# apple/ml-neuman

Hardware: AMD Instinct MI355X
Metric: rays_per_sec (800x800 frame, 128 samples/ray coarse + 128 importance, NeuMan background NeRF) (higher is better)
Workload: dtype coarse (sampling) pass: split-fp16 hi+lo MFMA x3, f32 accumulate; fine (shading) pass: per-row-scaled int16 as two int8 limbs on the i8 MFMA x3, exact int32 accumulate, encodings on split bf16

## Files before the change

include/neuman_hip.h:

```cpp
#ifndef NEUMAN_HIP_H
#define NEUMAN_HIP_H

#include <stdint.h>

#ifdef __cplusplus
extern "C" {
#endif

#define NM_OK 0
#define NM_ERR_ARG (-1)
#define NM_ERR_HIP (-2)
#define NM_ERR_UNSUPPORTED (-3)

#define NM_ABI_VERSION 1

typedef void* nm_stream_t;

#define NM_PREC_FP32 0
#define NM_PREC_BF16X3 1
#define NM_PREC_BF16 2
#define NM_PREC_I8X3 3
#define NM_PREC_FP16X3 4

#define NM_PE_POSENC 0
// ... 50 lines not shown
int nm_mlp_create(const nm_mlp_desc* desc, const float* const* host_params, const float* host_pos_tab,
                  const float* host_dir_tab, nm_mlp_t* out);
int nm_mlp_destroy(nm_mlp_t mlp);

int nm_mlp_forward(nm_mlp_t mlp, const float* pts, const float* dirs, int64_t n, int precision,
                   float sigma_scale, float* out, nm_stream_t stream);
int nm_mlp_refresh_f16(nm_mlp_t mlp, const float* const* dev_params, nm_stream_t stream);
int nm_mlp_forward_save(nm_mlp_t mlp, const float* pts, const float* dirs, int64_t n, float* save_h, float* save_hv,
                        float* out, nm_stream_t stream);
int nm_mlp_forward_save_bits(nm_mlp_t mlp, const float* pts, const float* dirs, int64_t n, float* save_h, float* save_hv,
                             uint32_t* save_bits, float* out, nm_stream_t stream);
int64_t nm_mlp_backward_chain_workspace_floats(int64_t n);
int nm_mlp_backward_chain(nm_mlp_t mlp, const float* const* dev_params, const float* dz_top, const float* d_feat, const float* d_raw,
                          const float* acts, const uint32_t* relu_bits, int64_t n, float* dz_out, float* bias_grads, float* workspace,
                          int64_t workspace_floats, nm_stream_t stream);
int nm_mlp_forward_save16(nm_mlp_t mlp, const float* pts, const float* dirs, int64_t n, uint16_t* save_h16, float* save_feat, uint16_t* save_feat16,
                          float* save_hv, uint32_t* save_bits, uint32_t* save_hvbits, uint16_t* save_x0h, uint16_t* save_d0h, float* out,
                          nm_stream_t stream);
int nm_mlp_backward_chain16(nm_mlp_t mlp, const float* const* dev_params, const float* d_feat, const float* d_raw, const uint32_t* relu_bits,
                            int64_t n, const float* amax, uint16_t* dz16, uint16_t* dfeat16, float* dz32_layer5, float* dz32_layer0,
                            float* bias_grads, float* workspace, int64_t workspace_floats, nm_stream_t stream);
int nm_mlp_backward_plain16(nm_mlp_t mlp, const float* const* dev_params, const float* d_out, const uint32_t* relu_bits, int64_t n, const float* amax,
                            uint16_t* dz16, float* dz32_layer5, float* dz32_layer0, float* bias_grads, float* workspace, int64_t workspace_floats,
                            nm_stream_t stream);
int nm_mlp_backward_net16(nm_mlp_t mlp, const float* const* dev_params, const float* d_raw, const float* d_feat_add, const uint32_t* relu_bits,
                          const uint32_t* hv_bits, int64_t n, const float* amax, uint16_t* dz16, uint16_t* dfeat16, uint16_t* dhv16, float* dz32_layer5, float* dz32_layer0,
                          float* dhv32, float* bias_grads, float* workspace, int64_t workspace_floats, nm_stream_t stream);
int nm_mlp_forward_rays(nm_mlp_t mlp, const float* origin, const float* direction, const float* z_vals,
                        int64_t R, int S, int precision, float sigma_scale, float* out, nm_stream_t stream);
#define NM_LIVE_CHUNK_SAMPLES (1 << 21)
int64_t nm_mlp_forward_rays_live_workspace_bytes(int64_t R, int S, int64_t chunk_samples);
int nm_mlp_forward_rays_live(nm_mlp_t mlp, const float* origin, const float* direction, const float* z_vals, int64_t R, int S, int precision,
                             float sigma_scale, float* out, void* workspace, int64_t workspace_bytes, int64_t chunk_samples, nm_stream_t stream);
int nm_mlp_sigma_rays(nm_mlp_t mlp, const float* origin, const float* direction, const float* z_vals,
                      int64_t R, int S, int precision, float sigma_scale, float* out, nm_stream_t stream);
int nm_mlp_forward_ray_chunk(nm_mlp_t mlp, const float* origin, const float* direction, const float* z_vals, int S_total,
                             const int32_t* ray_idx, const int32_t* n_rays_dev, int64_t n_rays, int s0, int S, int precision,
                             float sigma_scale, float* out, nm_stream_t stream);
int nm_mlp_sigma_ray_chunk(nm_mlp_t mlp, const float* origin, const float* direction, const float* z_vals, int S_total,
                           const int32_t* ray_idx, const int32_t* n_rays_dev, int64_t n_rays, int s0, int S, int precision,
                           float sigma_scale, float* out, nm_stream_t stream);
float nm_occ_probe_offset(int probes, int seed, int k, int axis);
int64_t nm_occ_build_workspace_floats(int res, int probes);
int nm_occ_build(nm_mlp_t mlp, const float* aabb, int res, int probes, int dilate, float sigma_threshold, int seed, int precision,
                 float* workspace, int64_t workspace_floats, uint32_t* bits, nm_stream_t stream);
int64_t nm_occ_compact_workspace_ints(int64_t n_samples);
int nm_occ_compact_samples(const uint32_t* bits, int res, const float* aabb, const float* origin, const float* direction, const float* z_vals,
                           int64_t R, int S, int32_t* sample_idx, int32_t* counts, int32_t* workspace, nm_stream_t stream);
int nm_mlp_forward_samples(nm_mlp_t mlp, const float* origin, const float* direction, const float* z_vals, int64_t R, int S,
                           const int32_t* sample_idx, const int32_t* n_dev, int64_t n_max, int precision, float sigma_scale, float* out,
                           nm_stream_t stream);
int nm_mlp_sigma_samples(nm_mlp_t mlp, const float* origin, const float* direction, const float* z_vals, int64_t R, int S,
                         const int32_t* sample_idx, const int32_t* n_dev, int64_t n_max, int precision, float sigma_scale, float* out,
                         nm_stream_t stream);
int nm_occ_compact_points(const uint32_t* bits, int res, const float* aabb, const float* pts, int64_t n, int32_t* point_idx, int32_t* counts,
                          int32_t* workspace, nm_stream_t stream);
int nm_mlp_forward_listed(nm_mlp_t mlp, const float* pts, const float* dirs, int64_t n_points, const int32_t* point_idx, const int32_t* n_dev,
                          int64_t n_max, int precision, float sigma_scale, float* out, nm_stream_t stream);
int64_t nm_mlp_live_workspace_bytes(int64_t n_max, int64_t chunk_samples);
int nm_mlp_forward_live(nm_mlp_t mlp, const float* pts, const float* dirs, int64_t n, int precision, float sigma_scale, float* out, void* workspace,
                        int64_t workspace_bytes, int64_t chunk_samples, nm_stream_t stream);
int nm_mlp_forward_listed_live(nm_mlp_t mlp, const float* pts, const float* dirs, int64_t n_points, const int32_t* point_idx, const int32_t* n_dev,
                               int64_t n_max, int precision, float sigma_scale, float* out, void* workspace, int64_t workspace_bytes,
                               int64_t chunk_samples, nm_stream_t stream);
int nm_mlp_forward_samples_live(nm_mlp_t mlp, const float* origin, const float* direction, const float* z_vals, int64_t R, int S,
                                const int32_t* sample_idx, const int32_t* n_dev, int64_t n_max, int precision, float sigma_scale, float* out,
// ... 166 lines not shown
```

ml-neuman_amd/csrc/mlp_host.hip:

```cpp
#include <math.h>
#include <stdarg.h>
#include <stdio.h>
#include <stdlib.h>
#include <string.h>

#include <algorithm>
#include <vector>

#include "common.h"
#include <string>
#include "mlp_layout.h"
#include "mlp_launch.h"

namespace nm {

static thread_local char g_err[512] = "";

void set_error(const char* fmt, ...) {
    va_list ap;
    va_start(ap, fmt);
    vsnprintf(g_err, sizeof(g_err), fmt, ap);
    va_end(ap);
}
int check_hip(hipError_t e, const char* what) {
// ... 945 lines not shown
    for (int i = 0; i < 24; ++i) {
        NM_REQUIRE(i >= 18 || dev_params[i], "nm_mlp_backward_plain16: dev_params[%d] is null", i);
        P.p[i] = i < 18 ? dev_params[i] : nullptr;
    }
    if (!m->d_bwd_image)
        if (int rc = nm::check_hip(hipMalloc(&m->d_bwd_image, (size_t)nm::mlp_bwd_image_bytes()), "nm_mlp_backward_plain16: hipMalloc")) return rc;
    nm::Bwd16 h;
    h.dz16 = dz16; h.dfeat16 = nullptr; h.amax = amax;
    for (int i = 0; i < 8; ++i) h.dz32[i] = nullptr;
    h.dz32[5] = dz32_layer5; h.dz32[0] = dz32_layer0;
    h.plain = 1;
    return nm::launch_mlp_bwd(P, 3 + 6 * m->desc.pos_n_freqs, m->d_bwd_image, nullptr, nullptr, d_out, nullptr, relu_bits, n, nullptr, workspace, bias_grads,
                              nm::as_stream(stream), &h);
}

int nm_mlp_forward_rays(nm_mlp_t mlp, const float* origin, const float* direction, const float* z_vals, int64_t R, int S,
                        int precision, float sigma_scale, float* out, nm_stream_t stream) {
    NM_REQUIRE(R == 0 || (origin && direction && z_vals && out), "nm_mlp_forward_rays: null pointer");
    NM_REQUIRE(R >= 0 && S >= 1, "nm_mlp_forward_rays: bad sizes");
    NM_REQUIRE((reinterpret_cast<uintptr_t>(out) & 15) == 0, "nm_mlp_forward_rays: out must be 16-byte aligned");
    return mlp_dispatch(mlp, nullptr, nullptr, origin, direction, z_vals, R * (int64_t)S, S, 1, precision, -2, sigma_scale, out,
                        nullptr, stream);
}

static int64_t live_chunk_rays(int64_t R, int S, int64_t chunk_samples) {
    if (chunk_samples <= 0) chunk_samples = NM_LIVE_CHUNK_SAMPLES;
    const int64_t rays = chunk_samples / S;
    return rays < 1 ? 1 : rays > R ? R : rays;
}
static int64_t live_cap(int64_t R, int S, int64_t chunk_samples) {
    return (live_chunk_rays(R, S, chunk_samples) * S + 255) / 256 * 256;
}

int64_t nm_mlp_forward_rays_live_workspace_bytes(int64_t R, int S, int64_t chunk_samples) {
    if (R < 0 || S < 1) return -1;
    return live_cap(R, S, chunk_samples) * (512 + 4 + 4) + 256;
}

int nm_mlp_forward_rays_live(nm_mlp_t m, const float* origin, const float* direction, const float* z_vals, int64_t R, int S, int precision,
                             float sigma_scale, float* out, void* workspace, int64_t workspace_bytes, int64_t chunk_samples, nm_stream_t stream) {
    NM_REQUIRE(m, "nm_mlp_forward_rays_live: null handle");
    if (m->desc.plain_head || precision != NM_PREC_I8X3 || !i8_as_kernel())
        return nm_mlp_forward_rays(m, origin, direction, z_vals, R, S, precision, sigma_scale, out, stream);
    NM_REQUIRE(R == 0 || (origin && direction && z_vals && out && workspace), "nm_mlp_forward_rays_live: null pointer");
    NM_REQUIRE(R >= 0 && S >= 1, "nm_mlp_forward_rays_live: bad sizes");
    NM_REQUIRE(((reinterpret_cast<uintptr_t>(out) | reinterpret_cast<uintptr_t>(workspace)) & 15) == 0, "nm_mlp_forward_rays_live: out and workspace must be 16-byte aligned");
    NM_REQUIRE(workspace_bytes >= nm_mlp_forward_rays_live_workspace_bytes(R, S, chunk_samples), "nm_mlp_forward_rays_live: workspace of %lld bytes, %lld needed",
               (long long)workspace_bytes, (long long)nm_mlp_forward_rays_live_workspace_bytes(R, S, chunk_samples));
    if (R == 0) return NM_OK;
    const int64_t cap = live_cap(R, S, chunk_samples), rays = live_chunk_rays(R, S, chunk_samples);
    NM_REQUIRE(rays * S < (1ll << 31), "nm_mlp_forward_rays_live: a chunk of %lld samples", (long long)(rays * S));
    nm::MlpLaunch L;
    L.wpack = nullptr; L.bias = nullptr; L.wpack16 = nullptr; L.bias16 = nullptr; L.wstream8 = nullptr;
    L.petab = m->d_petab;
    L.pe_kind = m->desc.pe_kind; L.pos_nfreq = m->desc.pos_n_freqs; L.dir_nfreq = m->desc.dir_n_freqs;
    L.pos_octaves = m->pos_octaves; L.dir_octaves = m->dir_octaves;
    L.plain_head = 0;
    L.consts8 = m->d_consts8;
    uint8_t* ws = static_cast<uint8_t*>(workspace);
    nm::LiveList live;
    live.x = reinterpret_cast<uint4*>(ws);
    live.sx = reinterpret_cast<float*>(ws + cap * 512);
    live.idx = reinterpret_cast<int*>(ws + cap * 516);
    live.count = reinterpret_cast<int*>(ws + cap * 520);
    live.cap = cap;
    hipStream_t st = nm::as_stream(stream);
    for (int64_t r0 = 0; r0 < R; r0 += rays) {
        const int64_t nr = R - r0 < rays ? R - r0 : rays;
        if (int rc = nm::check_hip(hipMemsetAsync(live.count, 0, 4, st), "nm_mlp_forward_rays_live: counter reset")) return rc;
        float* o = out + r0 * S * 4;
        if (int rc = nm::launch_mlp_i8s(L, m->d_trunk8, nullptr, nullptr, origin + r0 * 3, direction + r0 * 3, z_vals + r0 * S, nr * S, S, 1, sigma_scale, o, st,
                                        nullptr, &live))
            return rc;
        if (int rc = nm::launch_mlp_i8h(L, m->d_trunk8 + nm::kTrunkStreamBytes8, 3, nullptr, direction + r0 * 3, S, live, nr * S, o, st)) return rc;
    }
    return NM_OK;
}

int nm_mlp_sigma_rays(nm_mlp_t mlp, const float* origin, const float* direction, const float* z_vals, int64_t R, int S,
                      int precision, float sigma_scale, float* out, nm_stream_t stream) {
    NM_REQUIRE(R == 0 || (origin && direction && z_vals && out), "nm_mlp_sigma_rays: null pointer");
    NM_REQUIRE(R >= 0 && S >= 1, "nm_mlp_sigma_rays: bad sizes");
    NM_REQUIRE((reinterpret_cast<uintptr_t>(out) & 15) == 0, "nm_mlp_sigma_rays: out must be 16-byte aligned");
    return mlp_dispatch(mlp, nullptr, nullptr, origin, direction, z_vals, R * (int64_t)S, S, 1, precision, -2, sigma_scale, out,
                        nullptr, stream, nullptr, 1);
}

int nm_mlp_forward_ray_chunk(nm_mlp_t mlp, const float* origin, const float* direction, const float* z_vals, int S_total,
                             const int32_t* ray_idx, const int32_t* n_rays_dev, int64_t n_rays, int s0, int S, int precision,
                             float sigma_scale, float* out, nm_stream_t stream) {
    NM_REQUIRE(n_rays == 0 || (origin && direction && z_vals && ray_idx && out), "nm_mlp_forward_ray_chunk: null pointer");
// ... 215 lines not shown
```

ml-neuman_amd/csrc/mlp_launch.h:

```cpp
#pragma once
#include "common.h"

namespace nm {

enum { P_OUT_W = 16, P_OUT_B = 17 };
enum { P_PTS_W = 0, P_VIEWS_W = 16, P_VIEWS_B = 17, P_FEAT_W = 18, P_FEAT_B = 19, P_ALPHA_W = 20, P_ALPHA_B = 21, P_RGB_W = 22, P_RGB_B = 23 };
struct DevParams {
    const float* p[24];
};

struct MlpLaunch {
    const void* wpack; const float* bias; const float* petab;
    int pe_kind, pos_nfreq, dir_nfreq;
    int pos_octaves, dir_octaves;
    int plain_head;
    const void* wpack16; const float* bias16;
    const void* wstream8; const float* consts8;
    float* save_h = nullptr;
    float* save_hv = nullptr;
    unsigned* save_bits = nullptr;
    void* save_h16 = nullptr;
    void* save_feat16 = nullptr;
    unsigned* save_hvbits = nullptr;
    void* save_x0h = nullptr; void* save_d0h = nullptr;
};
struct RefLaunch {
    const float* wt; const float* bias; int off[12]; int boff[12]; const float* petab;
    int pe_kind, pos_nfreq, dir_nfreq;
    int plain_head;
};

struct MlpChunk {
    const int* ray_idx; const int* n_rays_dev; int s0, S_total;
};

int launch_mlp_mfma(const MlpLaunch& L, const float* pts, const float* dirs, const float* origin, const float* direction,
                    const float* z, int64_t n, int S, int in_mode, int precision, int stop_stage, float sigma_scale, float* out,
                    float* dbg, void* prof, hipStream_t stream, int sigma_only = 0, const MlpChunk* chunk = nullptr);
struct LiveList {
    uint4* x; float* sx; int* idx; int* count; int64_t cap;
};
int launch_mlp_i8s(const MlpLaunch& L, const void* image8, const float* pts, const float* dirs, const float* origin, const float* direction,
                   const float* z, int64_t n, int S, int in_mode, float sigma_scale, float* out, hipStream_t stream, const MlpChunk* chunk,
                   const LiveList* live = nullptr);
int launch_mlp_i8h(const MlpLaunch& L, const void* head8, int in_mode, const float* dirs, const float* direction, int S_total, const LiveList& live,
                   int64_t max_entries, float* out, hipStream_t stream);
int sigma_f16t_ndir();
int launch_sigma_f16t(const MlpLaunch& L, const void* stream16t, int stream_ndir, const float* pts, const float* dirs, const float* origin, const float* direction,
                      const float* z, int64_t n, int S, int in_mode, float sigma_scale, float* out, hipStream_t stream, const MlpChunk* chunk,
                      float* dbg, int dbg_stage);
int64_t mlp_bwd_image_bytes();
struct Bwd16 {
    void* dz16; void* dfeat16; const float* amax; float* dz32[8];
    const unsigned* hvbits = nullptr; void* dhv16 = nullptr; float* dhv32 = nullptr; int kdir = 0;
    int plain = 0;
};
int launch_mlp_bwd(const DevParams& P, int kpe, uint8_t* image, const float* dz_top, const float* d_feat, const float* d_raw, const float* acts,
                   const unsigned* relu_bits, int64_t n, float* dz_out, float* colsum, float* gb, hipStream_t stream, const Bwd16* h = nullptr);
int launch_mlp_ref(const RefLaunch& L, const float* pts, const float* dirs, const float* origin, const float* direction,
                   const float* z, int64_t n, int S, int in_mode, int stop_stage, float sigma_scale, float* out, float* dbg,
                   hipStream_t stream);

}
```

ml-neuman_amd/neuman_hip/_lib.py:

```python
import ctypes
import os

import torch

_HERE = os.path.dirname(os.path.abspath(__file__))
LIB_PATH = os.environ.get("NEUMAN_HIP_LIB") or os.path.join(_HERE, "..", "lib", "libneuman_hip.so")

c_f32p = ctypes.c_void_p
c_i32p = ctypes.c_void_p
c_stream = ctypes.c_void_p
i64 = ctypes.c_int64
i32 = ctypes.c_int

NM_PREC_FP32, NM_PREC_BF16X3, NM_PREC_BF16, NM_PREC_I8X3, NM_PREC_FP16X3 = 0, 1, 2, 3, 4
NM_PE_POSENC, NM_PE_ROTATE = 0, 1
PRECISIONS = {"fp32": NM_PREC_FP32, "bf16x3": NM_PREC_BF16X3, "bf16": NM_PREC_BF16, "i8x3": NM_PREC_I8X3, "fp16x3": NM_PREC_FP16X3}


class MlpDesc(ctypes.Structure):
    _fields_ = [("depth", ctypes.c_int32), ("width", ctypes.c_int32), ("skip", ctypes.c_int32),
                ("pe_kind", ctypes.c_int32), ("pos_n_freqs", ctypes.c_int32), ("dir_n_freqs", ctypes.c_int32),
                ("plain_head", ctypes.c_int32)]


# ... 21 lines not shown
    "nm_render_rays_human_occ": (i32, [ctypes.c_void_p, ctypes.c_void_p, ctypes.c_void_p, c_i32p, i32, ctypes.c_void_p, c_f32p, c_f32p, c_f32p, c_f32p, i64, i32,
                                       c_f32p, i32, ctypes.c_float, i32, c_f32p, c_f32p, c_f32p, c_i32p, c_f32p, c_f32p, c_f32p, c_stream]),
    "nm_compact_hits": (i32, [c_f32p, c_f32p, i64, c_i32p, c_i32p, c_i32p, c_i32p, c_stream]),
    "nm_mlp_pack_bytes": (i64, [ctypes.POINTER(MlpDesc)]),
    "nm_mlp_pack_i8s_bytes": (i64, [ctypes.POINTER(MlpDesc)]),
    "nm_mlp_pack_i8s": (i32, [ctypes.POINTER(MlpDesc), ctypes.POINTER(ctypes.c_void_p), ctypes.c_void_p]),
    "nm_mlp_pack_i8s_trunk_bytes": (i64, [ctypes.POINTER(MlpDesc)]),
    "nm_mlp_pack_i8s_head_bytes": (i64, [ctypes.POINTER(MlpDesc)]),
    "nm_mlp_pack_i8s_live": (i32, [ctypes.POINTER(MlpDesc), ctypes.POINTER(ctypes.c_void_p), ctypes.c_void_p, ctypes.c_void_p]),
    "nm_mlp_pack": (i32, [ctypes.POINTER(MlpDesc), ctypes.POINTER(ctypes.c_void_p), ctypes.c_void_p]),
    "nm_mlp_pack_f16": (i32, [ctypes.POINTER(MlpDesc), ctypes.POINTER(ctypes.c_void_p), ctypes.c_void_p]),
    "nm_mlp_pack_i8_bytes": (i64, [ctypes.POINTER(MlpDesc)]),
    "nm_mlp_pack_i8": (i32, [ctypes.POINTER(MlpDesc), ctypes.POINTER(ctypes.c_void_p), ctypes.c_void_p]),
    "nm_mlp_create": (i32, [ctypes.POINTER(MlpDesc), ctypes.POINTER(ctypes.c_void_p), ctypes.c_void_p, ctypes.c_void_p,
                            ctypes.POINTER(ctypes.c_void_p)]),
    "nm_mlp_destroy": (i32, [ctypes.c_void_p]),
    "nm_mlp_forward": (i32, [ctypes.c_void_p, c_f32p, c_f32p, i64, i32, ctypes.c_float, c_f32p, c_stream]),
    "nm_mlp_refresh_f16": (i32, [ctypes.c_void_p, ctypes.c_void_p, c_stream]),
    "nm_mlp_forward_save": (i32, [ctypes.c_void_p, c_f32p, c_f32p, i64, c_f32p, c_f32p, c_f32p, c_stream]),
    "nm_mlp_backward_chain_workspace_floats": (i64, [i64]),
    "nm_mlp_forward_save_bits": (i32, [ctypes.c_void_p, c_f32p, c_f32p, i64, c_f32p, c_f32p, ctypes.c_void_p, c_f32p, c_stream]),
    "nm_mlp_backward_chain": (i32, [ctypes.c_void_p, ctypes.c_void_p, c_f32p, c_f32p, c_f32p, c_f32p, ctypes.c_void_p, i64, c_f32p, c_f32p, c_f32p, i64, c_stream]),
    "nm_mlp_forward_save16": (i32, [ctypes.c_void_p, c_f32p, c_f32p, i64, ctypes.c_void_p, c_f32p, ctypes.c_void_p, c_f32p, ctypes.c_void_p, ctypes.c_void_p,
                                    ctypes.c_void_p, ctypes.c_void_p, c_f32p, c_stream]),
    "nm_mlp_backward_plain16": (i32, [ctypes.c_void_p, ctypes.c_void_p, c_f32p, ctypes.c_void_p, i64, c_f32p, ctypes.c_void_p, c_f32p, c_f32p, c_f32p, c_f32p, i64, c_stream]),
    "nm_mlp_backward_net16": (i32, [ctypes.c_void_p, ctypes.c_void_p, c_f32p, c_f32p, ctypes.c_void_p, ctypes.c_void_p, i64, c_f32p, ctypes.c_void_p, ctypes.c_void_p,
                                    ctypes.c_void_p, c_f32p, c_f32p, c_f32p, c_f32p, c_f32p, i64, c_stream]),
    "nm_mlp_backward_chain16": (i32, [ctypes.c_void_p, ctypes.c_void_p, c_f32p, c_f32p, ctypes.c_void_p, i64, c_f32p, ctypes.c_void_p, ctypes.c_void_p, c_f32p, c_f32p,
                                      c_f32p, c_f32p, i64, c_stream]),
    "nm_mlp_forward_rays": (i32, [ctypes.c_void_p, c_f32p, c_f32p, c_f32p, i64, i32, i32, ctypes.c_float, c_f32p, c_stream]),
    "nm_mlp_forward_rays_live_workspace_bytes": (i64, [i64, i32, i64]),
    "nm_mlp_forward_rays_live": (i32, [ctypes.c_void_p, c_f32p, c_f32p, c_f32p, i64, i32, i32, ctypes.c_float, c_f32p, ctypes.c_void_p, i64, i64, c_stream]),
    "nm_mlp_sigma_rays": (i32, [ctypes.c_void_p, c_f32p, c_f32p, c_f32p, i64, i32, i32, ctypes.c_float, c_f32p, c_stream]),
    "nm_mlp_live_workspace_bytes": (i64, [i64, i64]),
    "nm_mlp_forward_live": (i32, [ctypes.c_void_p, c_f32p, c_f32p, i64, i32, ctypes.c_float, c_f32p, ctypes.c_void_p, i64, i64, c_stream]),
    "nm_mlp_forward_listed_live": (i32, [ctypes.c_void_p, c_f32p, c_f32p, i64, c_i32p, c_i32p, i64, i32, ctypes.c_float, c_f32p, ctypes.c_void_p, i64, i64,
                                         c_stream]),
    "nm_mlp_forward_samples_live": (i32, [ctypes.c_void_p, c_f32p, c_f32p, c_f32p, i64, i32, c_i32p, c_i32p, i64, i32, ctypes.c_float, c_f32p, ctypes.c_void_p,
                                          i64, i64, c_stream]),
    "nm_mlp_forward_ray_chunk_live": (i32, [ctypes.c_void_p, c_f32p, c_f32p, c_f32p, i32, c_i32p, c_i32p, i64, i32, i32, i32, ctypes.c_float, c_f32p,
                                            ctypes.c_void_p, i64, i64, c_stream]),
    "nm_mlp_forward_ray_chunk": (i32, [ctypes.c_void_p, c_f32p, c_f32p, c_f32p, i32, c_i32p, c_i32p, i64, i32, i32, i32, ctypes.c_float, c_f32p,
                                       c_stream]),
    "nm_mlp_sigma_ray_chunk": (i32, [ctypes.c_void_p, c_f32p, c_f32p, c_f32p, i32, c_i32p, c_i32p, i64, i32, i32, i32, ctypes.c_float, c_f32p,
                                     c_stream]),
    "nm_transmittance_chunk": (i32, [c_f32p, c_f32p, c_f32p, c_i32p, c_i32p, i64, i32, i32, i32, c_f32p, c_stream]),
    "nm_transmittance_chunk_dz": (i32, [c_f32p, c_f32p, c_f32p, c_i32p, c_i32p, i64, i32, i32, i32, c_f32p, c_stream]),
    "nm_mlp_sigma_f16t_debug": (i32, [ctypes.c_void_p, c_f32p, c_f32p, i64, i32, c_f32p, c_f32p, c_stream]),
    "nm_mlp_forward_debug": (i32, [ctypes.c_void_p, c_f32p, c_f32p, i64, i32, i32, c_f32p, c_stream]),
    "nm_mlp_forward_profile": (i32, [ctypes.c_void_p, c_f32p, c_f32p, i64, i32, c_f32p, ctypes.c_void_p, c_stream]),
    "nm_mesh_create": (i32, [c_f32p, i32, c_i32p, i32, i32, ctypes.POINTER(ctypes.c_void_p), c_stream]),
    "nm_mesh_update": (i32, [ctypes.c_void_p, c_f32p, c_stream]),
    "nm_mesh_destroy": (i32, [ctypes.c_void_p]),
    "nm_mesh_info": (i32, [ctypes.c_void_p, ctypes.c_void_p, ctypes.c_void_p, ctypes.c_void_p]),
    "nm_warp_to_canonical": (i32, [ctypes.c_void_p, c_f32p, i64, i32, ctypes.c_void_p, c_f32p, c_f32p, c_f32p, c_stream]),
    "nm_warp_apply_forward": (i32, [c_f32p, c_i32p, c_f32p, c_f32p, i64, c_f32p, c_stream]),
    "nm_warp_apply_backward": (i32, [c_f32p, c_i32p, c_f32p, c_f32p, c_f32p, i64, i64, c_f32p, c_f32p, c_stream]),
    "nm_bary_forward": (i32, [c_f32p, c_i32p, c_f32p, i64, c_f32p, c_stream]),
    "nm_bary_backward": (i32, [c_f32p, c_i32p, c_f32p, c_f32p, i64, i64, c_f32p, c_stream]),
    "nm_smpl_create": (i32, [c_f32p, c_f32p, c_f32p, c_i32p, c_f32p, c_f32p, i32, i32, i32, ctypes.POINTER(ctypes.c_void_p)]),
    "nm_smpl_destroy": (i32, [ctypes.c_void_p]),
    "nm_smpl_vertex_workspace_floats": (i64, [ctypes.c_void_p]),
    "nm_smpl_vertex_forward": (i32, [ctypes.c_void_p, c_f32p, c_f32p, ctypes.c_void_p, ctypes.c_double, c_f32p, c_f32p, c_f32p, c_f32p, c_stream]),
    "nm_smpl_vertex_backward": (i32, [ctypes.c_void_p, c_f32p, c_f32p, ctypes.c_void_p, ctypes.c_double, c_f32p, c_f32p, c_f32p, c_f32p, c_f32p,
                                      c_f32p, c_f32p, c_stream]),
    "nm_smpl_frames": (i32, [ctypes.c_void_p, c_f32p, c_f32p, ctypes.c_void_p, i32, ctypes.c_double, i32, ctypes.c_void_p, c_f32p, c_f32p,
# ... 111 lines not shown
```

ml-neuman_amd/neuman_hip/vanilla.py:

```python
import contextlib
import ctypes
import os

import numpy as np
import torch
import torch.nn as nn

from . import _lib

DEFAULT_PRECISION = os.environ.get("NEUMAN_PRECISION", "mixed")


def weight_reset(m):
    if isinstance(m, nn.Linear):
        m.reset_parameters()


class Embedder(nn.Module):

    def __init__(self, input_dims, max_freq, N_freqs, log_sampling=True, include_input=True, min_freq=0, mapping='posenc'):
        super().__init__()
        if mapping not in ('posenc', 'rotate'):
            raise ValueError(mapping)
        assert log_sampling or mapping == 'rotate', "log_sampling=False is not a configuration of the reference (models/vanilla.py:70)"
# ... 209 lines not shown
            from . import train
            if sigma_scale != 1.0:
                raise _lib.NeumanHipError("sigma_scale is a render-time option (render_utils.py:229)")
            return train.mlp_forward_train(self, input_pts, input_views)
        self._guard(input_pts, input_views)
        shp = input_pts.shape[:-1]
        p = input_pts.detach().reshape(-1, 3).contiguous()
        d = input_views.detach().reshape(-1, 3).contiguous()
        out = torch.empty((p.shape[0], 4), device=p.device, dtype=torch.float32)
        if self.live_route(precision, role, p.shape[0]):
            ws, nbytes = live_workspace_for(p.shape[0], chunk_samples, p.device)
            _lib.check(_lib.lib().nm_mlp_forward_live(self.handle(), _lib.dev_ptr(p, name='input_pts'), _lib.dev_ptr(d, name='input_views'), p.shape[0],
                                                      self._prec(precision, role), float(sigma_scale), _lib.dev_ptr(out), _lib.dev_ptr(ws, torch.uint8), nbytes,
                                                      int(chunk_samples), _lib.stream_ptr()), "nm_mlp_forward_live")
            return out.reshape(*shp, 4)
        _lib.check(_lib.lib().nm_mlp_forward(self.handle(), _lib.dev_ptr(p, name='input_pts'), _lib.dev_ptr(d, name='input_views'),
                                             p.shape[0], self._prec(precision, role), float(sigma_scale), _lib.dev_ptr(out),
                                             _lib.stream_ptr()), "nm_mlp_forward")
        return out.reshape(*shp, 4)

    def forward_two_views(self, input_pts, input_views, other_views):
        from . import train
        n = input_pts.reshape(-1, input_pts.shape[-1]).shape[0]
        if not (self.training and torch.is_grad_enabled() and self.nerf.use_viewdirs and self.pos_pe.input_dims == 3 and train.two_views_ok(self, n)):
            return None
        return train.two_views(self, input_pts, input_views, other_views)

    def forward_rays(self, origin, direction, z_vals, precision=None, sigma_scale=1.0, role=None, sigma_only=False, chunk_samples=0):
        self._guard(origin, direction, z_vals)
        R, S = z_vals.shape
        out = torch.empty((R, S, 4), device=z_vals.device, dtype=torch.float32)
        if role == 'composite' and not sigma_only and self.nerf.use_viewdirs and self._prec(precision, role) == _lib.NM_PREC_I8X3:
            nbytes = int(_lib.lib().nm_mlp_forward_rays_live_workspace_bytes(R, S, int(chunk_samples)))
            ws, _ = live_workspace_for(R * S, chunk_samples, z_vals.device, nbytes)
            _lib.check(_lib.lib().nm_mlp_forward_rays_live(
                self.handle(), _lib.dev_ptr(origin, name='origin'), _lib.dev_ptr(direction, name='direction'), _lib.dev_ptr(z_vals, name='z_vals'), R, S,
                self._prec(precision, role), float(sigma_scale), _lib.dev_ptr(out), _lib.dev_ptr(ws, torch.uint8), nbytes, int(chunk_samples),
                _lib.stream_ptr()), "nm_mlp_forward_rays_live")
            return out
        entry = _lib.lib().nm_mlp_sigma_rays if sigma_only else _lib.lib().nm_mlp_forward_rays
        _lib.check(entry(self.handle(), _lib.dev_ptr(origin, name='origin'), _lib.dev_ptr(direction, name='direction'),
                         _lib.dev_ptr(z_vals, name='z_vals'), R, S, self._prec(precision, role), float(sigma_scale),
                         _lib.dev_ptr(out), _lib.stream_ptr()), "nm_mlp_sigma_rays" if sigma_only else "nm_mlp_forward_rays")
        return out

    def forward_ray_chunk(self, origin, direction, z_vals, ray_idx, n_rays_dev, s0, chunk, out, precision=None, sigma_scale=1.0, role=None,
                          sigma_only=False, chunk_samples=0):
        self._guard(origin, direction, z_vals)
        R, S = z_vals.shape
        n = ray_idx.shape[0] * int(chunk)
        if self.live_route(precision, role, n, sigma_only) and R * S < (1 << 31):
            ws, nbytes = live_workspace_for(n, chunk_samples, z_vals.device)
            _lib.check(_lib.lib().nm_mlp_forward_ray_chunk_live(
                self.handle(), _lib.dev_ptr(origin, name='origin'), _lib.dev_ptr(direction, name='direction'), _lib.dev_ptr(z_vals, name='z_vals'), S,
                _lib.dev_ptr(ray_idx, torch.int32, 'ray_idx'), _lib.dev_ptr(n_rays_dev, torch.int32, 'n_rays_dev'), ray_idx.shape[0], int(s0), int(chunk),
                self._prec(precision, role), float(sigma_scale), _lib.dev_ptr(out), _lib.dev_ptr(ws, torch.uint8), nbytes, int(chunk_samples),
                _lib.stream_ptr()), "nm_mlp_forward_ray_chunk_live")
            return out
        entry = _lib.lib().nm_mlp_sigma_ray_chunk if sigma_only else _lib.lib().nm_mlp_forward_ray_chunk
        _lib.check(entry(
            self.handle(), _lib.dev_ptr(origin, name='origin'), _lib.dev_ptr(direction, name='direction'), _lib.dev_ptr(z_vals, name='z_vals'), S,
            _lib.dev_ptr(ray_idx, torch.int32, 'ray_idx'), _lib.dev_ptr(n_rays_dev, torch.int32, 'n_rays_dev'), ray_idx.shape[0], int(s0), int(chunk),
            self._prec(precision, role), float(sigma_scale), _lib.dev_ptr(out), _lib.stream_ptr()), "nm_mlp_forward_ray_chunk")
        return out

    def forward_debug(self, input_pts, input_views, stage, precision=None):
# ... 108 lines not shown
```

Before: 1.507 million.

## Fuse trunk and color-head passes into one persistent kernel with per-block live lists

Adds a persistent fused kernel that runs the int8 trunk on sample tiles, appends samples with positive density into a per-workgroup ring list in global memory, and runs the color head on batches of those listed samples inside the same block. The weight ring stream switches between trunk and head images according to which phase comes next. This replaces the earlier separate trunk and head launches with their global compaction, cutting launch and compaction overhead and avoiding head work on dead samples. The cost is a larger workspace, a grid limited to the CU count, and a list that can wrap if too many entries are pending.

```diff
diff --git a/include/neuman_hip.h b/include/neuman_hip.h
--- a/include/neuman_hip.h
+++ b/include/neuman_hip.h
@@ -106,6 +106,10 @@
 int64_t nm_mlp_forward_rays_live_workspace_bytes(int64_t R, int S, int64_t chunk_samples);
 int nm_mlp_forward_rays_live(nm_mlp_t mlp, const float* origin, const float* direction, const float* z_vals, int64_t R, int S, int precision,
                              float sigma_scale, float* out, void* workspace, int64_t workspace_bytes, int64_t chunk_samples, nm_stream_t stream);
+#define NM_LIVE_FUSED_DEFAULT 1
+int64_t nm_mlp_live_fused_workspace_bytes(int64_t n);
+int nm_mlp_forward_rays_fused(nm_mlp_t mlp, const float* origin, const float* direction, const float* z_vals, int64_t R, int S, float sigma_scale,
+                              float* out, void* workspace, int64_t workspace_bytes, nm_stream_t stream);
 int nm_mlp_sigma_rays(nm_mlp_t mlp, const float* origin, const float* direction, const float* z_vals,
                       int64_t R, int S, int precision, float sigma_scale, float* out, nm_stream_t stream);
 int nm_mlp_forward_ray_chunk(nm_mlp_t mlp, const float* origin, const float* direction, const float* z_vals, int S_total,
diff --git a/ml-neuman_amd/csrc/mlp_host.hip b/ml-neuman_amd/csrc/mlp_host.hip
--- a/ml-neuman_amd/csrc/mlp_host.hip
+++ b/ml-neuman_amd/csrc/mlp_host.hip
@@ -1001,6 +1001,37 @@
     return (live_chunk_rays(R, S, chunk_samples) * S + 255) / 256 * 256;
 }
 
+static bool live_fused() {
+    const char* e = getenv("NEUMAN_LIVE_FUSED");
+    return e ? !strcmp(e, "1") : NM_LIVE_FUSED_DEFAULT != 0;
+}
+static void live_launch(nm_mlp_t m, nm::MlpLaunch& L) {
+    L.wpack = nullptr; L.bias = nullptr; L.wpack16 = nullptr; L.bias16 = nullptr; L.wstream8 = nullptr;
+    L.petab = m->d_petab;
+    L.pe_kind = m->desc.pe_kind; L.pos_nfreq = m->desc.pos_n_freqs; L.dir_nfreq = m->desc.dir_n_freqs;
+    L.pos_octaves = m->pos_octaves; L.dir_octaves = m->dir_octaves;
+    L.plain_head = 0;
+    L.consts8 = m->d_consts8;
+}
+
+int64_t nm_mlp_live_fused_workspace_bytes(int64_t n) { return n < 0 ? -1 : nm::fused_workspace_bytes(n); }
+
+int nm_mlp_forward_rays_fused(nm_mlp_t m, const float* origin, const float* direction, const float* z_vals, int64_t R, int S, float sigma_scale, float* out,
+                              void* workspace, int64_t workspace_bytes, nm_stream_t stream) {
+    NM_REQUIRE(((reinterpret_cast<uintptr_t>(out) | reinterpret_cast<uintptr_t>(workspace)) & 15) == 0, "nm_mlp_forward_rays_fused: out and workspace must be 16-byte aligned");
+    NM_REQUIRE(R >= 0 && S >= 1 && R < (1ll << 31) && R * (int64_t)S < (1ll << 31), "nm_mlp_forward_rays_fused: bad sizes (R=%lld S=%d)", (long long)R, S);
+    const int64_t need = nm::fused_workspace_bytes(R * (int64_t)S);
+    NM_REQUIRE((workspace || R == 0) && workspace_bytes >= need, "nm_mlp_forward_rays_fused: workspace of %lld bytes, %lld needed", (long long)workspace_bytes, (long long)need);
+    NM_REQUIRE(R == 0 || (origin && direction && z_vals && out), "nm_mlp_forward_rays_fused: null pointer");
+    NM_REQUIRE(m, "nm_mlp_forward_rays_fused: null handle");
+    NM_REQUIRE(!m->desc.plain_head && i8_as_kernel(), "nm_mlp_forward_rays_fused: no such kernel for the plain-head net or under NEUMAN_I8_KERNEL=w");
+    if (R == 0) return NM_OK;
+    nm::MlpLaunch L;
+    live_launch(m, L);
+    return nm::launch_mlp_i8f(L, m->d_trunk8, (int)nm::kTrunkStreamBytes8, origin, direction, z_vals, R * (int64_t)S, S, sigma_scale, out, workspace,
+                              nm::as_stream(stream));
+}
+
 int64_t nm_mlp_forward_rays_live_workspace_bytes(int64_t R, int S, int64_t chunk_samples) {
     if (R < 0 || S < 1) return -1;
     return live_cap(R, S, chunk_samples) * (512 + 4 + 4) + 256;
@@ -1020,12 +1051,10 @@
     const int64_t cap = live_cap(R, S, chunk_samples), rays = live_chunk_rays(R, S, chunk_samples);
     NM_REQUIRE(rays * S < (1ll << 31), "nm_mlp_forward_rays_live: a chunk of %lld samples", (long long)(rays * S));
     nm::MlpLaunch L;
-    L.wpack = nullptr; L.bias = nullptr; L.wpack16 = nullptr; L.bias16 = nullptr; L.wstream8 = nullptr;
-    L.petab = m->d_petab;
-    L.pe_kind = m->desc.pe_kind; L.pos_nfreq = m->desc.pos_n_freqs; L.dir_nfreq = m->desc.dir_n_freqs;
-    L.pos_octaves = m->pos_octaves; L.dir_octaves = m->dir_octaves;
-    L.plain_head = 0;
-    L.consts8 = m->d_consts8;
+    live_launch(m, L);
+    if (live_fused() && R * (int64_t)S < (1ll << 31) && workspace_bytes >= nm::fused_workspace_bytes(R * (int64_t)S))
+        return nm::launch_mlp_i8f(L, m->d_trunk8, (int)nm::kTrunkStreamBytes8, origin, direction, z_vals, R * (int64_t)S, S, sigma_scale, out, workspace,
+                                  nm::as_stream(stream));
     uint8_t* ws = static_cast<uint8_t*>(workspace);
     nm::LiveList live;
     live.x = reinterpret_cast<uint4*>(ws);
diff --git a/ml-neuman_amd/csrc/mlp_i8f.hip b/ml-neuman_amd/csrc/mlp_i8f.hip
--- /dev/null
+++ b/ml-neuman_amd/csrc/mlp_i8f.hip
@@ -0,0 +1,307 @@
+#include "mlp_i8as.h"
+
+namespace {
+
+constexpr int kTrunkSteps = 8 * 4 + 7 * 8 * 8 + 8 * 4 + 8;
+constexpr int kHeadSteps = 8 * 8 + 4 * 10 + 4;
+struct TrunkStream {
+    static __host__ __device__ constexpr int steps(int i) { return i < 8 ? 4 : 8; }
+};
+struct HeadStream {
+    static __host__ __device__ constexpr int steps(int i) {
+        i = i >= 13 ? i - 13 : i;
+        return i < 8 ? 8 : i < 12 ? 10 : 4;
+    }
+};
+
+struct ArgsF {
+    MlpArgs a;
+    const float* consts8;
+    const char* image;
+    int head_off;
+    char* list;
+    int* tiles;
+};
+
+struct RingF {
+    const char* src;
+    const uint4* rd;
+    unsigned lds0;
+    int off, slot;
+    int refill, np, nsteps2;
+    int edge, next;
+};
+__device__ __forceinline__ void ring_piece(const RingF& R, int off, int slot, int j) {
+    glds16(R.src + off + j * (kWaves * 1024), __builtin_amdgcn_readfirstlane(R.lds0 + slot * (kSlotU4 * 16) + j * (kWaves * 1024)));
+}
+template <class S>
+__device__ __forceinline__ const uint4* ring_enter_f(RingF& R, int i) {
+    const int np1 = block_pieces(S::steps(i + 1));
+    if (np1 == 1) asm volatile("s_waitcnt vmcnt(1)" ::: "memory");
+    else if (np1 == 2) asm volatile("s_waitcnt vmcnt(2)" ::: "memory");
+    else asm volatile("s_waitcnt vmcnt(3)" ::: "memory");
+    __builtin_amdgcn_s_barrier();
+    const uint4* cur = R.rd + R.slot * kSlotU4;
+    R.refill = R.slot == 0 ? kSlots - 1 : R.slot - 1;
+    R.slot = R.slot == kSlots - 1 ? 0 : R.slot + 1;
+    R.np = block_pieces(S::steps(i + 2));
+    R.nsteps2 = S::steps(i + 2);
+    return cur;
+}
+__device__ __forceinline__ void ring_copy(RingF& R, int j) {
+    if (j < R.np) ring_piece(R, R.off, R.refill, j);
+    if (j == R.np - 1) {
+        R.off += R.nsteps2 * nm::kStepBytes;
+        if (R.off == R.edge) R.off = R.next;
+    }
+}
+
+__global__ __launch_bounds__(kWaves * 64, 2) void nerf_mlp_i8s_fused_kernel(const ArgsF A) {
+    __shared__ uint4 lds[kPeU4 + kSlots * kSlotU4 + kBiasU4];
+    __shared__ float units[4];
+    __shared__ unsigned appended;
+    const MlpArgs a = A.a;
+    const int tid = threadIdx.x, lane = tid & 63;
+    const int w = __builtin_amdgcn_readfirstlane(tid >> 6);
+    const int g = lane >> 5, s = lane & 31;
+    uint4* pw = lds + w * kPWaveU4;
+    RingF R;
+    R.src = A.image + lane * 16 + w * 1024;
+    R.rd = lds + kPeU4 + lane;
+    R.lds0 = (unsigned)(uintptr_t)(lds + kPeU4) + w * 1024;
+    R.slot = 0;
+    {
+        float* lb = reinterpret_cast<float*>(lds + kPeU4 + kSlots * kSlotU4);
+        for (int i = tid; i < nm::kBiasFloats + 16; i += kWaves * 64) lb[i] = A.consts8[nm::kBiasFloats + i];
+    }
+    if (tid == 0) appended = 0;
+    if (tid < 4) units[tid] = A.consts8[tid == 0 ? nm::stage_b_off(8) + 256 : nm::stage_b_off(10) + tid - 1];
+    __syncthreads();
+    ring_piece(R, 0, 0, 0);
+    ring_piece(R, 4 * nm::kStepBytes, 1, 0);
+    const float* kappa = reinterpret_cast<const float*>(lds + kPeU4 + kSlots * kSlotU4) + nm::kBiasFloats;
+    unsigned bias_lds = (unsigned)(uintptr_t)(lds + kPeU4 + kSlots * kSlotU4) + 16 * g;
+    asm volatile("" : "+v"(bias_lds));
+    lds_cfloat* bias = (lds_cfloat*)(uintptr_t)bias_lds;
+    const int64_t ntiles = (a.n + kTile - 1) / kTile;
+    for (int i = lane; i < kPWaveU4; i += 64) pw[i] = make_uint4(0, 0, 0, 0);
+    char* const mine = A.list + (int64_t)blockIdx.x * nm::kFusedListBytes;
+    uint4* const lx = reinterpret_cast<uint4*>(mine);
+    float* const lsx = reinterpret_cast<float*>(mine + nm::kFusedEntries * 512);
+    int* const lidx = reinterpret_cast<int*>(mine + nm::kFusedEntries * 516);
+
+    int64_t tile = blockIdx.x;
+    unsigned consumed = 0;
+    int head = 0, ntrunk = 0, nhead = 0;
+#pragma unroll 1
+    for (;;) {
+        __builtin_amdgcn_fence(__ATOMIC_RELEASE, "workgroup");
+        __builtin_amdgcn_s_barrier();
+        __builtin_amdgcn_fence(__ATOMIC_ACQUIRE, "workgroup");
+        const unsigned pending = (unsigned)__builtin_amdgcn_readfirstlane(__hip_atomic_load(&appended, __ATOMIC_RELAXED, __HIP_MEMORY_SCOPE_WORKGROUP)) - consumed;
+        if (head && pending == 0) break;
+        const unsigned ntake = head ? (pending < (unsigned)kTile ? pending : (unsigned)kTile) : 0u;
+        const bool more = (head ? tile : tile + gridDim.x) < ntiles;
+        const int next_head = pending - ntake >= (unsigned)kTile || !more;
+        R.off = head ? A.head_off + 16 * nm::kStepBytes : 8 * nm::kStepBytes;
+        R.edge = head ? A.head_off + kHeadSteps * nm::kStepBytes : kTrunkSteps * nm::kStepBytes;
+        R.next = next_head ? A.head_off : kTrunkSteps * nm::kStepBytes;
+        asm volatile("" : "+s"(R.off), "+s"(R.edge), "+s"(R.next));
+        if (!head) {
+            const int64_t row0 = tile * kTile + w * kRows;
+            fill_pe_wave(pw, false, a, row0, lane);
+            X8 X;
+            float sx;
+            {
+                f32x16 f[8];
+                float m = 0.f;
+#pragma unroll
+                for (int b = 0; b < 8; ++b) {
+                    const uint4* ws = ring_enter_f<TrunkStream>(R, b);
+                    bias16(f[b], bias + nm::stage_b_off(0) + 32 * b);
+                    k_bf<4, true>(f[b], pw, g, s, ws, &R);
+                    m = max16<true>(m, f[b]);
+                }
+                const float M = row_max(m), inv = inv_of(M);
+#pragma unroll
+                for (int b = 0; b < 8; ++b) quant16<true>(f[b], inv, X.h[b], X.l[b]);
+                sx = scale_of(M);
+            }
+#pragma unroll 1
+            for (int st = 1; st <= 7; ++st) {
+                const float sxin = sx * (256.f * kappa[st]);
+                const int i0 = 8 * st + (st > 5 ? 4 : 0);
+                f32x16 f[8];
+                float m = 0.f;
+                i32x16 tp;
+#pragma unroll
+                for (int b = 0; b < 8; ++b) {
+                    const uint4* ws = ring_enter_f<TrunkStream>(R, i0 + b);
+                    if (b == 0) {
+                        k_i8<8>(tp, X, ws, R);
+                    } else {
+                        i32x16 t;
+                        k_i8_impl<8, true>(t, X, ws, R, f[b - 1], tp, bias + 256 * st + 32 * (b - 1), sxin, m);
+                        tp = t;
+                    }
+                }
+                dequant16(f[7], tp, sxin, bias + 256 * st + 32 * 7);
+                if (st == 5) {
+#pragma unroll
+                    for (int u = 0; u < 4; ++u) {
+                        const uint4* ws = ring_enter_f<TrunkStream>(R, 48 + u);
+                        k_bf<4, true>(f[2 * u], pw, g, s, ws, &R, 0);
+                        k_bf<4, true>(f[2 * u + 1], pw, g, s, ws + 4 * kStepU4, &R, 2);
+                    }
+                    m = 0.f;
+#pragma unroll
+                    for (int b = 0; b < 7; ++b) m = max16<true>(m, f[b]);
+                }
+                m = max16<true>(m, f[7]);
+                const float M = row_max(m), inv = inv_of(M);
+#pragma unroll
+                for (int b = 0; b < 8; ++b) quant16<true>(f[b], inv, X.h[b], X.l[b]);
+                sx = scale_of(M);
+            }
+            {
+                i32x16 t;
+                f32x16 fa;
+                k_i8<8>(t, X, ring_enter_f<TrunkStream>(R, 68), R);
+                dequant16(fa, t, sx * (256.f * kappa[8]), bias + nm::stage_b_off(8) + 256);
+                const float sigma = fa[0] * units[0];
+                const float v = sigma * a.sigma_scale;
+                int sb = s, gb = g;
+                asm volatile("" : "+v"(sb), "+v"(gb));
+                const int64_t i = row0 + s;
+                if (g == 0 && i < a.n) reinterpret_cast<float4*>(a.out)[i] = make_float4(0.f, 0.f, 0.f, v);
+                const unsigned live = (unsigned)__builtin_amdgcn_ballot_w64(g == 0 && i < a.n && !(v <= 0.f));
+                if (live) {
+                    unsigned base = 0;
+                    if (lane == 0) base = __hip_atomic_fetch_add(&appended, (unsigned)__builtin_popcount(live), __ATOMIC_RELAXED, __HIP_MEMORY_SCOPE_WORKGROUP);
+                    base = (unsigned)__builtin_amdgcn_readfirstlane(base);
+                    if ((live >> sb) & 1) {
+                        const unsigned e = (base + __builtin_popcount(live & ((1u << sb) - 1u))) % (unsigned)nm::kFusedEntries;
+                        uint4* dst = lx + gb * nm::kFusedEntries + e;
+#pragma unroll
+                        for (int k = 0; k < 8; ++k) {
+                            dst[(4 * k) * nm::kFusedEntries] = X.h[k];
+                            dst[(4 * k + 2) * nm::kFusedEntries] = X.l[k];
+                        }
+                        if (g == 0) { lsx[e] = sx; lidx[e] = (int)i; }
+                    }
+                }
+            }
+            tile += gridDim.x;
+            ++ntrunk;
+        } else {
+            const unsigned e0 = consumed % (unsigned)nm::kFusedEntries;
+            MlpArgs ah = a;
+            ah.in_mode = 3;
+            ah.ray_idx = lidx + e0;
+            ah.n = ntake;
+            ah.s0 = 0;
+            ah.S_total = a.S;
+            const int64_t row0 = w * kRows;
+            int e = w * kRows + s;
+            const bool listed = e < (int)ntake;
+            if (!listed) e = (int)ntake - 1;
+            X8 X;
+            {
+                const uint4* src = lx + g * nm::kFusedEntries + e0 + e;
+#pragma unroll
+                for (int k = 0; k < 8; ++k) {
+                    X.h[k] = src[(4 * k) * nm::kFusedEntries];
+                    X.l[k] = src[(4 * k + 2) * nm::kFusedEntries];
+                }
+            }
+            float sx = lsx[e0 + e];
+            int rec = lidx[e0 + e];
+            fill_pe_wave(pw, true, ah, row0, lane);
+            asm volatile("" : "+v"(rec));
+            {
+                const float sxin = sx * (256.f * kappa[8]);
+                f32x16 f[8];
+                float m = 0.f;
+#pragma unroll
+                for (int b = 0; b < 8; ++b) {
+                    i32x16 t;
+                    k_i8<8>(t, X, ring_enter_f<HeadStream>(R, b), R);
+                    dequant16(f[b], t, sxin, bias + nm::stage_b_off(8) + 32 * b);
+                    m = max16<false>(m, f[b]);
+                }
+                const float M = row_max(m), inv = inv_of(M);
+#pragma unroll
+                for (int b = 0; b < 8; ++b) quant16<false>(f[b], inv, X.h[b], X.l[b]);
+                sx = scale_of(M);
+            }
+            {
+                const float sxin = sx * (256.f * kappa[9]);
+                f32x16 f[4];
+                float m = 0.f;
+#pragma unroll
+                for (int b = 0; b < 4; ++b) {
+                    i32x16 t;
+                    const uint4* ws = ring_enter_f<HeadStream>(R, 8 + b);
+                    k_i8<8>(t, X, ws, R);
+                    dequant16(f[b], t, sxin, bias + nm::stage_b_off(9) + 32 * b);
+                    k_bf<2>(f[b], pw, g, s, ws + 8 * kStepU4);
+                    m = max16<true>(m, f[b]);
+                }
+                const float M = row_max(m), inv = inv_of(M);
+#pragma unroll
+                for (int b = 0; b < 4; ++b) quant16<true>(f[b], inv, X.h[b], X.l[b]);
+                sx = scale_of(M);
+            }
+            {
+                i32x16 t;
+                f32x16 fr;
+                k_i8<4>(t, X, ring_enter_f<HeadStream>(R, 12), R);
+                dequant16(fr, t, sx * (256.f * kappa[10]), bias + nm::stage_b_off(10));
+                if (g == 0 && listed) {
+                    float* o = a.out + (int64_t)rec * 4;
+                    o[0] = fr[0] * units[1]; o[1] = fr[1] * units[2]; o[2] = fr[2] * units[3];
+                }
+            }
+            consumed += ntake;
+            ++nhead;
+        }
+        head = next_head;
+    }
+    if (tid == 0) { A.tiles[2 * blockIdx.x] = ntrunk; A.tiles[2 * blockIdx.x + 1] = nhead; }
+    asm volatile("s_waitcnt vmcnt(0)" ::: "memory");
+}
+
+}
+
+namespace nm {
+
+int launch_mlp_i8f(const MlpLaunch& L, const void* trunk8, int head_off, const float* origin, const float* direction, const float* z, int64_t n, int S,
+                   float sigma_scale, float* out, void* workspace, hipStream_t stream) {
+    ArgsF A;
+    MlpArgs& a = A.a;
+    a.ray_idx = nullptr; a.n_rays_dev = nullptr; a.s0 = 0; a.S_total = S;
+    a.wpack = nullptr; a.bias = nullptr;
+    a.petab = L.petab;
+    a.pts = nullptr; a.dirs = nullptr; a.origin = origin; a.direction = direction; a.z = z;
+    a.out = out; a.dbg = nullptr; a.prof = nullptr; a.n = n; a.S = S; a.in_mode = 1; a.stop_stage = -2; a.sigma_scale = sigma_scale;
+    a.sigma_only = 0;
+    a.save_h = nullptr; a.save_hv = nullptr; a.save_bits = nullptr; a.save_h16 = nullptr; a.save_feat16 = nullptr; a.save_hvbits = nullptr; a.save_x0h = nullptr; a.save_d0h = nullptr;
+    a.pos = PeSpec{L.pe_kind, L.pos_nfreq, L.pos_octaves};
+    a.dir = PeSpec{L.pe_kind, L.dir_nfreq, L.dir_octaves};
+    A.consts8 = L.consts8;
+    A.image = static_cast<const char*>(trunk8);
+    A.head_off = head_off;
+    const int64_t groups = fused_groups(n);
+    A.list = static_cast<char*>(workspace);
+    A.tiles = reinterpret_cast<int*>(A.list + groups * kFusedListBytes);
+    int dev = 0, cus = kFusedMaxGroups;
+    if (hipGetDevice(&dev) == hipSuccess) {
+        int v = 0;
+        if (hipDeviceGetAttribute(&v, hipDeviceAttributeMultiprocessorCount, dev) == hipSuccess && v > 0) cus = v;
+    }
+    const int grid = (int)(groups < cus ? groups : cus);
+    hipLaunchKernelGGL(nerf_mlp_i8s_fused_kernel, dim3(grid), dim3(kWaves * 64), 0, stream, A);
+    return check_launch("nerf_mlp_i8s_fused_kernel");
+}
+
+}
diff --git a/ml-neuman_amd/csrc/mlp_launch.h b/ml-neuman_amd/csrc/mlp_launch.h
--- a/ml-neuman_amd/csrc/mlp_launch.h
+++ b/ml-neuman_amd/csrc/mlp_launch.h
@@ -45,6 +45,15 @@
                    const LiveList* live = nullptr);
 int launch_mlp_i8h(const MlpLaunch& L, const void* head8, int in_mode, const float* dirs, const float* direction, int S_total, const LiveList& live,
                    int64_t max_entries, float* out, hipStream_t stream);
+constexpr int kFusedEntries = 768, kFusedMaxGroups = 256;
+constexpr int64_t kFusedListBytes = (int64_t)kFusedEntries * (512 + 4 + 4);
+inline int64_t fused_groups(int64_t n) {
+    const int64_t tiles = (n + 255) / 256;
+    return tiles < kFusedMaxGroups ? tiles : kFusedMaxGroups;
+}
+inline int64_t fused_workspace_bytes(int64_t n) { return fused_groups(n) * kFusedListBytes + (fused_groups(n) * 8 + 255) / 256 * 256; }
+int launch_mlp_i8f(const MlpLaunch& L, const void* trunk8, int head_off, const float* origin, const float* direction, const float* z, int64_t n, int S,
+                   float sigma_scale, float* out, void* workspace, hipStream_t stream);
 int sigma_f16t_ndir();
 int launch_sigma_f16t(const MlpLaunch& L, const void* stream16t, int stream_ndir, const float* pts, const float* dirs, const float* origin, const float* direction,
                       const float* z, int64_t n, int S, int in_mode, float sigma_scale, float* out, hipStream_t stream, const MlpChunk* chunk,
diff --git a/ml-neuman_amd/neuman_hip/_lib.py b/ml-neuman_amd/neuman_hip/_lib.py
--- a/ml-neuman_amd/neuman_hip/_lib.py
+++ b/ml-neuman_amd/neuman_hip/_lib.py
@@ -77,6 +77,8 @@
     "nm_mlp_forward_rays_live_workspace_bytes": (i64, [i64, i32, i64]),
     "nm_mlp_forward_rays_live": (i32, [ctypes.c_void_p, c_f32p, c_f32p, c_f32p, i64, i32, i32, ctypes.c_float, c_f32p, ctypes.c_void_p, i64, i64, c_stream]),
     "nm_mlp_sigma_rays": (i32, [ctypes.c_void_p, c_f32p, c_f32p, c_f32p, i64, i32, i32, ctypes.c_float, c_f32p, c_stream]),
+    "nm_mlp_live_fused_workspace_bytes": (i64, [i64]),
+    "nm_mlp_forward_rays_fused": (i32, [ctypes.c_void_p, c_f32p, c_f32p, c_f32p, i64, i32, ctypes.c_float, c_f32p, ctypes.c_void_p, i64, c_stream]),
     "nm_mlp_live_workspace_bytes": (i64, [i64, i64]),
     "nm_mlp_forward_live": (i32, [ctypes.c_void_p, c_f32p, c_f32p, i64, i32, ctypes.c_float, c_f32p, ctypes.c_void_p, i64, i64, c_stream]),
     "nm_mlp_forward_listed_live": (i32, [ctypes.c_void_p, c_f32p, c_f32p, i64, c_i32p, c_i32p, i64, i32, ctypes.c_float, c_f32p, ctypes.c_void_p, i64, i64,
diff --git a/ml-neuman_amd/neuman_hip/vanilla.py b/ml-neuman_amd/neuman_hip/vanilla.py
--- a/ml-neuman_amd/neuman_hip/vanilla.py
+++ b/ml-neuman_amd/neuman_hip/vanilla.py
@@ -265,6 +265,8 @@
         out = torch.empty((R, S, 4), device=z_vals.device, dtype=torch.float32)
         if role == 'composite' and not sigma_only and self.nerf.use_viewdirs and self._prec(precision, role) == _lib.NM_PREC_I8X3:
             nbytes = int(_lib.lib().nm_mlp_forward_rays_live_workspace_bytes(R, S, int(chunk_samples)))
+            if R * S < (1 << 31):
+                nbytes = max(nbytes, int(_lib.lib().nm_mlp_live_fused_workspace_bytes(R * S)))
             ws, _ = live_workspace_for(R * S, chunk_samples, z_vals.device, nbytes)
             _lib.check(_lib.lib().nm_mlp_forward_rays_live(
                 self.handle(), _lib.dev_ptr(origin, name='origin'), _lib.dev_ptr(direction, name='direction'), _lib.dev_ptr(z_vals, name='z_vals'), R, S,
```

Result: faster. 1.528 million (median of 6 runs) (+1.4%).
